# MatejBevec/gcn-song-embeddings

Hardware: AMD Instinct MI355X
Metric: PinSAGE train-step nodes/sec (2-hop, batch 512) at 1/2/4/8 MI355X (higher is better)
Workload: dtype f32

## Files before the change

gcn-song-embeddings_amd/csrc/capi.hip:

```cpp
#include <hip/hip_runtime.h>

#include <algorithm>
#include <cstdlib>
#include <cstring>
#include <string>
#include <vector>

#include "../../include/pinsage_hip.h"
#include "aggw.h"
#include "als.h"
#include "bpr.h"
#include "lmf.h"
#include "n2v.h"
#include "sage.h"
#include "capi.h"
#include "conv.h"
#include "cooc.h"
#include "dq.h"
#include "fly.h"
#include "frontier.h"
#include "gemm.h"
#include "knn.h"
#include "listmetrics.h"
#include "ppr_topk.h"
// ... 606 lines not shown
                 splits >= 0 && scratch && A3 && B3 && a3_ps >= 0 && b3_ps >= 0,
             kErrArg, "wgrad_planes: bad argument");
  KwParams p;
  p.A3 = A3;
  p.a3_ps = a3_ps;
  p.lda = lda;
  p.M = (int)M;
  p.B3 = B3;
  p.b3_ps = b3_ps;
  p.ldb = ldb;
  p.b_idx = b_idx;
  p.N = (int)N;
  p.K_dev = K_dev;
  p.K_max = (int)K_max;
  p.dst = dst;
  p.ld_dst = ld_dst;
  p.dst_b = dst_b;
  char* sc = static_cast<char*>(scratch);
  p.cnt = reinterpret_cast<int*>(sc);
  sc += align_up(wgrad_kw_tickets((int)M, (int)N) * 4, 256);
  p.slab = reinterpret_cast<float*>(sc);
  sc += wgrad_kw_slab_floats((int)M, (int)N) * 4;
  p.bslab = reinterpret_cast<float*>(sc);
  p.S = splits;
  return launch_wgrad_kw(p, (hipStream_t)stream);
}

int pinsage_gemm_ex(int64_t M, int64_t N, int64_t K, int a_kmajor, int b_kmajor, const float* A,
                    int64_t lda, const int32_t* a_idx, const float* B, int64_t ldb,
                    const int32_t* b_idx, float* C, int64_t ldc, const float* bias, int act,
                    int epi, int splits, int cfg, int stream_k, void* stream) {
  if (M < 0 || N <= 0 || K < 0 || M > INT32_MAX || N > INT32_MAX || K > INT32_MAX ||
      (epi != kEpiStore && epi != kEpiAccum && epi != kEpiPartial) || splits < 1 || cfg < -1 ||
      cfg > 5) {
    set_error("gemm_ex: bad argument");
    return kErrArg;
  }
  GemmParams p;
  p.M = (int)M;
  p.N = (int)N;
  p.K = (int)K;
  p.a_kmajor = a_kmajor != 0;
  p.b_kmajor = b_kmajor != 0;
  p.a = A;
  p.lda = lda;
  p.a_idx = a_idx;
  p.b = B;
  p.ldb = ldb;
  p.b_idx = b_idx;
  p.c = C;
  p.ldc = ldc;
  p.bias = bias;
  p.act = act != 0;
  p.epi = epi;
  p.splits = splits;
  p.cfg = cfg;
  p.stream_k = stream_k;
  if (cfg == 5 && (!gemm_ws_supported(p) || stream_k == 1 || gemm_default_prec() != 1)) {
    set_error("gemm_ex: cfg 5 needs split-bf16 products, K-major A and B, a store epilogue, K % 32 == 0, "
              "N % 128 == 0 and no stream-K");
    return kErrArg;
  }
  if (stream_k != 0) {
    static float* slab = nullptr;
    static int* cnt = nullptr;
    constexpr int64_t kCnt = 1 << 20;
    if (!slab) {
// ... 53 lines not shown
                       int64_t M_max, int64_t K, const float* W, const uint16_t* W_ilv, int64_t ldw_ilv,
                       const float* bias, int64_t N, int act, float* C, int64_t ldc, void* stream) {
  if (M < 0 || N <= 0 || K <= 0 || M > INT32_MAX || N > INT32_MAX || K > INT32_MAX || M_max < 0 ||
      M_max > INT32_MAX || (M_dev && M_max == 0)) {
    set_error("linear_ilv: bad argument");
    return kErrArg;
  }
  GemmParams p;
  p.M = (int)M;
  p.M_dev = M_dev;
  p.M_max = (int)M_max;
  p.N = (int)N;
  p.K = (int)K;
  p.a_ilv = A_ilv;
  p.lda_ilv = lda_ilv;
  p.a_idx = a_idx;
  p.b = W;
  p.ldb = K;
  p.b_ilv = W_ilv;
  p.ldb_ilv = W_ilv ? ldw_ilv : 0;
  p.c = C;
  p.ldc = ldc;
  p.bias = bias;
  p.act = act != 0;
  p.prec = 1;
  return launch_gemm(p, (hipStream_t)stream);
}

int pinsage_linear_split_b(const float* A, int64_t lda, const int32_t* a_idx, int64_t M, int64_t K,
                           const float* W, const uint16_t* W_planes, int64_t ldws,
                           const float* bias, int64_t N, int act, float* C, int64_t ldc, int cfg,
                           void* stream) {
  if (M < 0 || N <= 0 || K < 0 || M > INT32_MAX || N > INT32_MAX || K > INT32_MAX || cfg < -1 ||
      cfg > 5) {
    set_error("linear_split_b: bad argument");
    return kErrArg;
  }
  if (ldws != K) {
    set_error("linear_split_b: W_planes must come from pinsage_split_planes(W, N, K, ...): ldws == K");
    return kErrArg;
  }
  GemmParams p;
  p.M = (int)M;
  p.N = (int)N;
  p.K = (int)K;
  p.a = A;
  p.lda = lda;
  p.a_idx = a_idx;
  p.b = W;
  p.ldb = K;
  p.b_split = W_planes;
  p.ldb_split = ldws;
  p.c = C;
  p.ldc = ldc;
  p.bias = bias;
  p.act = act != 0;
  p.cfg = cfg;
  p.stream_k = 0;
  p.prec = 1;
  return launch_gemm(p, (hipStream_t)stream);
}

int64_t pinsage_cooc_tile(void) { return cooc_tile(); }

int64_t pinsage_cooc_scratch_bytes(int64_t n_tracks, int64_t batch_rows) {
  return cooc_scratch_bytes(n_tracks, batch_rows < 1 ? 1 : batch_rows);
}
// ... 307 lines not shown
  p.b = W;
  p.ldb = d + hid;
  p.c = y;
  p.ldc = out;
  p.bias = bias;
  p.epi = kEpiL2Norm;
  p.norms = norms;
  p.stream_k = 0;
  return launch_gemm(p, (hipStream_t)stream);
}

int pinsage_norm_lrelu_backward(const float* y, const float* norms, const float* dy, int64_t n, int64_t out,
                                float* dp, void* stream) {
  if (n < 0 || out <= 0 || out > INT32_MAX) {
    set_error("norm_lrelu_backward: bad sizes");
    return kErrArg;
  }
  if (n == 0) return kOk;
  return launch_norm_lrelu_bwd(y, norms, dy, (int)out, nullptr, n, dp, nullptr, 0, nullptr, nullptr, 0,
                               (hipStream_t)stream);
}

int64_t pinsage_gemm_sk_slab_floats(void) { return gemm_sk_slab_floats(); }

int pinsage_gemm_params(const pinsage_gemm_params_t* q, int* ran_stream_k, void* stream) {
  if (ran_stream_k) *ran_stream_k = 0;
  PS_REQUIRE(q && q->size == (int64_t)sizeof(pinsage_gemm_params_t), kErrArg,
             "gemm_params: null or a struct of another size");
  auto fits = [](int64_t v) { return v >= -1 && v <= INT32_MAX; };
  PS_REQUIRE(fits(q->M) && fits(q->N) && fits(q->K) && fits(q->M_max) && fits(q->K_max) && fits(q->K1) &&
                 fits(q->N1) && fits(q->splits) && fits(q->M_hint) && fits(q->sk_min_units) && q->M >= 0 &&
                 q->K >= 0 && q->M_max >= 0 && q->K_max >= 0 && q->splits >= 1 && q->M_hint >= 0,
             kErrArg, "gemm_params: a size out of range");
  PS_REQUIRE(q->epi >= kEpiStore && q->epi <= kEpiPartial && q->cfg >= -1 && q->cfg <= 5 && q->stream_k >= -1 &&
                 q->stream_k <= 1 && q->prec >= -1 && q->prec <= 1,
             kErrArg, "gemm_params: epi 0..3, cfg -1..5, stream_k -1..1, prec -1..1");
  PS_REQUIRE((q->a || q->a_ilv) && (q->b || q->b_ilv) && q->c, kErrArg, "gemm_params: a, b and c must be set");
  PS_REQUIRE((q->sk_slab != nullptr) == (q->sk_cnt != nullptr) && (!q->sk_cnt || q->sk_cnt_len > 0), kErrArg,
             "gemm_params: stream-K scratch needs the slab, the tickets and their count");
  GemmParams p;
  p.M = (int)q->M;
  p.N = (int)q->N;
  p.K = (int)q->K;
  p.M_dev = q->M_dev;
  p.K_dev = q->K_dev;
  p.M_max = (int)q->M_max;
  p.K_max = (int)q->K_max;
  p.a_kmajor = q->a_kmajor != 0;
  p.b_kmajor = q->b_kmajor != 0;
  p.a = q->a;
  p.lda = q->lda;
  p.a_idx = q->a_idx;
  p.K1 = (int)q->K1;
  p.a2 = q->a2;
  p.lda2 = q->lda2;
  p.a2_idx = q->a2_idx;
  p.b = q->b;
  p.ldb = q->ldb;
  p.b_idx = q->b_idx;
  p.N1 = (int)q->N1;
  p.b2 = q->b2;
  p.ldb2 = q->ldb2;
  p.b2_idx = q->b2_idx;
  p.c = q->c;
  p.ldc = q->ldc;
  p.c_idx = q->c_idx;
  p.c2 = q->c2;
  p.ldc2 = q->ldc2;
  p.bias_part = q->bias_part;
// ... 140 lines not shown
```

gcn-song-embeddings_amd/csrc/engine.hip:

```cpp
#include <hip/hip_runtime.h>

#include <algorithm>
#include <cstdlib>
#include <cstring>
#include <deque>
#include <functional>
#include <map>
#include <mutex>
#include <atomic>
#include <string>
#include <vector>

#include "aggw.h"
#include "common.h"
#include "conv.h"
#include "dq.h"
#include "frontier.h"
#include "gemm.h"
#include "head.h"
#include "wgrad.h"

namespace ps {

struct EngineConfig {
// ... 1173 lines not shown
  return kOk;
}

int pinsage_engine_read_counts(const pinsage_engine* e, void* ws, int64_t* S, int64_t* N,
                               void* stream) {
  const Engine* E = reinterpret_cast<const Engine*>(e);
  PS_CHECK_HIP(hipStreamSynchronize((hipStream_t)stream));
  for (size_t l = 0; l < E->L.size(); ++l) {
    int v = 0;
    PS_CHECK_HIP(hipMemcpy(&v, at<int>(ws, E->L[l].S.count), 4, hipMemcpyDeviceToHost));
    S[l] = v;
    PS_CHECK_HIP(hipMemcpy(&v, at<int>(ws, E->L[l].N.count), 4, hipMemcpyDeviceToHost));
    N[l] = v;
  }
  return kOk;
}

int pinsage_engine_set_frontier_fork(pinsage_engine* e, int on) {
  if (!e) {
    set_error("engine_set_frontier_fork: null engine");
    return kErrArg;
  }
  reinterpret_cast<Engine*>(e)->frontier_fork_ok = on != 0;
  return kOk;
}

int pinsage_engine_set_gemm_choice(pinsage_engine* e, const char* site, int cfg, int stream_k,
                                   int splits) {
  Engine* E = reinterpret_cast<Engine*>(e);
  if (!E || !site) {
    set_error("engine_set_gemm_choice: null argument");
    return kErrArg;
  }
  if (cfg < -1 || cfg > 5 || stream_k < -1 || stream_k > 1 || splits < 0 || splits > kMaxSplits) {
    set_error("engine_set_gemm_choice: cfg in [-1, 5], stream_k in [-1, 1], splits in [0, 64]");
    return kErrArg;
  }
  if (cfg < 0 && stream_k < 0 && splits == 0) E->choice.erase(site);
  else E->choice[site] = Engine::GemmChoice{cfg, stream_k, splits};
  return kOk;
}

int pinsage_engine_site_stream_k(const pinsage_engine* e, const char* site) {
  const Engine* E = reinterpret_cast<const Engine*>(e);
  if (!E || !site) return -1;
  auto it = E->sk_used.find(site);
  return it == E->sk_used.end() ? -1 : it->second;
}

int pinsage_engine_set_layer_table(pinsage_engine* e, int64_t layer, const int32_t* nb,
                                   const float* wn, int64_t ld) {
  Engine* E = reinterpret_cast<Engine*>(e);
  if (!E || layer < 0 || layer >= E->cfg.n_layers || ((nb == nullptr) != (wn == nullptr)) ||
      (nb && ld < E->cfg.T)) {
    set_error("engine_set_layer_table: bad argument");
    return kErrArg;
  }
  LayerBuf& lb = E->L[(size_t)layer];
  lb.nb_tab = nb;
  lb.wn_tab = wn;
  lb.ld_tab = ld;
  return kOk;
}

int pinsage_engine_set_hints(pinsage_engine* e, const int64_t* S, const int64_t* N) {
  Engine* E = reinterpret_cast<Engine*>(e);
  for (size_t l = 0; l < E->L.size(); ++l) {
    E->L[l].S.hint = S ? S[l] : 0;
// ... 191 lines not shown
```

gcn-song-embeddings_amd/csrc/gemm.h:

```cpp
#pragma once
#include "common.h"

namespace ps {

enum GemmEpi : int {
  kEpiStore = 0,
  kEpiAccum = 1,
  kEpiL2Norm = 2,
  kEpiPartial = 3,
};

struct GemmParams {
  int M = 0, N = 0, K = 0;
  const int* M_dev = nullptr;
  const int* K_dev = nullptr;
  int M_max = 0, K_max = 0;
  bool a_kmajor = true, b_kmajor = true;
  const float* a = nullptr;
  int64_t lda = 0;
  const int32_t* a_idx = nullptr;
  int K1 = -1;
  const float* a2 = nullptr;
  int64_t lda2 = 0;
  const int32_t* a2_idx = nullptr;
// ... 18 lines not shown
  float* norms = nullptr;
  int splits = 1;
  int M_hint = 0;
  int cfg = -1;
  float* sk_slab = nullptr;
  int* sk_cnt = nullptr;
  int64_t sk_cnt_len = 0;
  int stream_k = -1;
  int sk_min_units = 4;
  int prec = -1;
  const uint16_t* b_split = nullptr;
  int64_t ldb_split = 0;
  const uint16_t* a_ilv = nullptr;
  const uint16_t* b_ilv = nullptr;
  int64_t lda_ilv = 0, ldb_ilv = 0;
};

int launch_split_ilv(const float* src, int64_t ld, int64_t rows, int K, uint16_t* out, int64_t ldo, hipStream_t st);

int launch_split_planes(const float* w, int64_t rows, int64_t cols, int64_t ldw, uint16_t* out,
                        hipStream_t st);

int gemm_default_prec();
void gemm_set_default_prec(int prec);

int64_t gemm_sk_slab_floats();
int gemm_slots();

int gemm_pick_config(int M, int N, int K, int splits);

int launch_gemm(const GemmParams& p, hipStream_t st);
int gemm_last_stream_k();
bool gemm_ws_supported(const GemmParams& p);

}
```

gcn-song-embeddings_amd/csrc/gemm.hip:

```cpp
#include "gemm.h"

#include <algorithm>

#include "bf16split.h"
#include "lds_dma.h"
#include <type_traits>

namespace ps {

typedef float f32x16 __attribute__((ext_vector_type(16)));

constexpr int kLdsBudget = 81920;
constexpr int kLdsBudget3 = 54272;
constexpr int kLdsBudget4 = 40960;
constexpr int kIdxWin = 1024;

__device__ __forceinline__ void zero16(float* l) {
  *reinterpret_cast<float4*>(l) = make_float4(0.f, 0.f, 0.f, 0.f);
}

template <int R, int BK>
struct KOp {
  static constexpr int CPR = BK / 4;
  static constexpr int NI = R * CPR / 256;
  static constexpr int SZ = R * BK;
  static_assert(R * CPR % 256 == 0, "whole DMAs per thread");
  static constexpr int SH = BK == 32 ? 1 : 2;
  __device__ static __forceinline__ int swz(int row) { return (row >> SH) & (CPR - 1); }
  __device__ static __forceinline__ float4 frag(const float* img, int row, int k4) {
    return *reinterpret_cast<const float4*>(img + row * BK + 4 * ((k4 >> 2) ^ swz(row)));
  }
  const float* rp[NI];
  const float* rp2[NI];
  int lc[NI];
  __device__ __forceinline__ void init(int tid, int r0, int rmax, const float* a, int64_t lda,
                                       const int32_t* idx, const float* a2, int64_t lda2,
                                       const int32_t* idx2) {
#pragma unroll
    for (int j = 0; j < NI; ++j) {
      const int q = j * 256 + tid, row = q / CPR;
      lc[j] = 4 * ((q % CPR) ^ swz(row));
      const int g = r0 + row, rc = g < rmax ? g : rmax - 1;
      rp[j] = a + (int64_t)(idx ? idx[rc] : rc) * lda;
// ... 100 lines not shown
      base = a2 + (cl - c1);
      ld = lda2;
      gathered = idx2 != nullptr;
    } else {
      base = a + cl;
      ld = lda;
      gathered = idx != nullptr;
    }
  }
  __device__ __forceinline__ void issue(unsigned img, int wave, int k0, int kend, const int* sidx,
                                        int wb) const {
#pragma unroll
    for (int j = 0; j < NI; ++j) {
      const int k = min(k0 + kr0 + KSTEP * j, kend - 1);
      const int64_t r = gathered ? sidx[k - wb] : k;
      glds16(base + r * ld, img + (unsigned)(j * 256 + wave * 64) * 16u);
    }
  }
  __device__ __forceinline__ void zero_tail(float* img, int tid, int k0, int kend) const {
#pragma unroll
    for (int j = 0; j < NI; ++j)
      if (k0 + kr0 + KSTEP * j >= kend) zero16(img + (j * 256 + tid) * 4);
  }
};

struct SkPlan {
  int64_t U;
  int I, Ga;
  __device__ __forceinline__ int64_t start(int b) const { return (int64_t)b * U / Ga; }
  __device__ __forceinline__ int block_of(int64_t u) const {
    return (int)(((u + 1) * Ga - 1) / U);
  }
};

__device__ __forceinline__ float dpp_xor1(float x) {
  return __int_as_float(__builtin_amdgcn_mov_dpp(__float_as_int(x), 0xB1, 0xF, 0xF, false));
}
__device__ __forceinline__ float dpp_xor2(float x) {
  return __int_as_float(__builtin_amdgcn_mov_dpp(__float_as_int(x), 0x4E, 0xF, 0xF, false));
}
__device__ __forceinline__ void quad_transpose16(float (&v)[16], int lane) {
  const int i = lane & 3;
#pragma unroll
  for (int g = 0; g < 4; ++g) {
    float t[4];
#pragma unroll
    for (int k = 0; k < 4; ++k) t[k] = dpp_xor1(v[4 * g + (k ^ 1)]);
#pragma unroll
    for (int k = 0; k < 4; ++k)
      if ((i & 1) != (k & 1)) v[4 * g + k] = t[k];
#pragma unroll
    for (int k = 0; k < 4; ++k) t[k] = dpp_xor2(v[4 * g + (k ^ 2)]);
#pragma unroll
    for (int k = 0; k < 4; ++k)
      if ((i & 2) != (k & 2)) v[4 * g + k] = t[k];
  }
}

template <bool AK, bool BKM, int WM, int WN, int TM, int TN, int BK, int NSMAX = 4, int WPC = 2,
          bool BF = false, bool PB = false, bool SK = true, int IL = 0>
__global__ __launch_bounds__(256, WPC) void gemm_f32_kernel(GemmParams p) {
  static_assert(!BF || BK % 16 == 0, "split-bf16 products: 16-k steps");
  static_assert(!PB || (BF && BKM), "pre-split B: split-bf16 products, K-major B");
  static_assert(!IL || (BF && AK && BKM && !PB && !SK && BK == 16), "interleaved planes: split bf16, K-major A and B");
  constexpr int BM = WM * TM * 32, BN = WN * TN * 32;
  using OpA = typename std::conditional<
      IL != 0, IlvOp<BM>, typename std::conditional<AK, KOp<BM, BK>, MNOp<BM, BK>>::type>::type;
  using OpBp = typename std::conditional<
      PB, KSplitOp<BN, BK>, typename std::conditional<BKM, KOp<BN, BK>, MNOp<BN, BK>>::type>::type;
  using OpB = typename std::conditional<IL == 1, IlvOp<BN>, OpBp>::type;
  constexpr int SZA = OpA::SZ, SZB = OpB::SZ, SZS = SZA + SZB;
  constexpr int NG = OpA::NI + OpB::NI;
  constexpr bool GA = !AK, GB = !BKM;
  constexpr int IDXF = (GA ? kIdxWin : 0) + (GB ? kIdxWin : 0);
  constexpr int NSA = ((WPC == 2 ? kLdsBudget : WPC == 3 ? kLdsBudget3 : kLdsBudget4) / 4 - IDXF) / SZS;
  constexpr int NS = NSA > NSMAX ? NSMAX : NSA;
  static_assert(NS >= 3, "stage buffers do not fit");
  __shared__ __attribute__((aligned(16))) float smem[NS * SZS + IDXF];
  int* const sidxA = reinterpret_cast<int*>(smem + NS * SZS);
  int* const sidxB = sidxA + (GA ? kIdxWin : 0);

  const int tid = threadIdx.x, lane = tid & 63, wave = tid >> 6;
  const int wm = wave / WN, wn = wave % WN;
#ifdef PS_GEMM_PROBE
  uint64_t pt[6] = {__builtin_amdgcn_s_memrealtime(), 0, 0, 0, 0, 0};
  int pti = 1;
#define PS_PROBE() do { if (pti < 6) pt[pti++] = __builtin_amdgcn_s_memrealtime(); } while (0)
#else
#define PS_PROBE() do { } while (0)
#endif
// ... 275 lines not shown
          for (int o = 1; o < 32; o <<= 1) s2 += __shfl_xor(s2, o, 64);
          if (l32 == 0) red[wn * BM + (wm * TM + i) * 32 + (r & 3) + 8 * (r >> 2) + 4 * h] = s2;
        }
      __syncthreads();
#pragma unroll
      for (int i = 0; i < TM; ++i) {
        int64_t dsts[16];
#pragma unroll
        for (int r = 0; r < 16; ++r) {
          const int row = m0 + (wm * TM + i) * 32 + (r & 3) + 8 * (r >> 2) + 4 * h;
          dsts[r] = row < M ? (p.c_idx ? (int64_t)p.c_idx[row] : (int64_t)row) : -1;
        }
#pragma unroll
        for (int r = 0; r < 16; ++r) asm volatile("" : "+v"(dsts[r]));
#pragma unroll
        for (int r = 0; r < 16; ++r) {
          const int lrow = (wm * TM + i) * 32 + (r & 3) + 8 * (r >> 2) + 4 * h;
          const int row = m0 + lrow;
          if (row >= M) continue;
          float tot = 0.f;
#pragma unroll
          for (int q = 0; q < WN; ++q) tot += red[q * BM + lrow];
          const float nrm = sqrtf(tot);
          const int64_t dst = dsts[r];
#pragma unroll
          for (int j = 0; j < TN; ++j) {
            const int col = n0 + (wn * TN + j) * 32 + l32;
            if (col < N) p.c[dst * p.ldc + col] = acc[i][j][r] / nrm;
          }
          if (p.norms && wn == 0 && l32 == 0) p.norms[row] = nrm;
        }
      }
    } else {
      const bool accum = p.epi == kEpiAccum;
      const bool wide = N % 4 == 0 && p.ldc % 4 == 0 && (reinterpret_cast<uintptr_t>(p.c) & 15) == 0 &&
                        (!p.c2 || (p.ldc2 % 4 == 0 && p.N1 % 4 == 0 && (reinterpret_cast<uintptr_t>(p.c2) & 15) == 0)) &&
                        (!p.mask || (p.ldm % 4 == 0 && (reinterpret_cast<uintptr_t>(p.mask) & 15) == 0));
      if (wide) {
#pragma unroll
        for (int i = 0; i < TM; ++i)
#pragma unroll
          for (int j = 0; j < TN; ++j) {
            float v[16];
#pragma unroll
            for (int r = 0; r < 16; ++r) {
              float x = acc[i][j][r] + bj[j];
              if (p.act) x = lrelu(x);
              v[r] = x;
            }
            quad_transpose16(v, lane);
            const int col = n0 + (wn * TN + j) * 32 + 4 * (l32 >> 2);
            const bool second = p.c2 && col >= p.N1;
            int rows[4];
            int64_t dst[4];
#pragma unroll
            for (int g = 0; g < 4; ++g) {
              rows[g] = m0 + (wm * TM + i) * 32 + (l32 & 3) + 8 * g + 4 * h;
              dst[g] = rows[g] < M && col < N ? (p.c_idx ? (int64_t)p.c_idx[rows[g]] : (int64_t)rows[g]) : -1;
            }
            float4 pre[4];
#pragma unroll
            for (int g = 0; g < 4; ++g) {
              pre[g] = make_float4(0.f, 0.f, 0.f, 0.f);
              if (dst[g] >= 0) {
                if (p.mask) pre[g] = *reinterpret_cast<const float4*>(p.mask + (int64_t)rows[g] * p.ldm + col);
                else if (accum && !second) pre[g] = *reinterpret_cast<const float4*>(p.c + dst[g] * p.ldc + col);
              }
            }
            float4 val[4];
#pragma unroll
            for (int g = 0; g < 4; ++g) {
              float4 x = make_float4(v[4 * g], v[4 * g + 1], v[4 * g + 2], v[4 * g + 3]);
              if (p.mask) {
                x.x *= lrelu_grad(pre[g].x);
                x.y *= lrelu_grad(pre[g].y);
                x.z *= lrelu_grad(pre[g].z);
                x.w *= lrelu_grad(pre[g].w);
              } else if (accum && !second) {
                x.x = pre[g].x + x.x;
                x.y = pre[g].y + x.y;
                x.z = pre[g].z + x.z;
                x.w = pre[g].w + x.w;
              }
              val[g] = x;
              asm volatile("" : "+v"(val[g].x), "+v"(val[g].y), "+v"(val[g].z), "+v"(val[g].w));
            }
#pragma unroll
            for (int g = 0; g < 4; ++g)
              if (dst[g] >= 0)
                *reinterpret_cast<float4*>(second ? p.c2 + (int64_t)rows[g] * p.ldc2 + (col - p.N1)
                                                  : p.c + dst[g] * p.ldc + col) = val[g];
          }
      } else {
#pragma unroll
      for (int i = 0; i < TM; ++i)
#pragma unroll
        for (int r0 = 0; r0 < 16; r0 += 8) {
          int dsts[8];
#pragma unroll
          for (int r = 0; r < 8; ++r) {
            const int row = m0 + (wm * TM + i) * 32 + ((r0 + r) & 3) + 8 * ((r0 + r) >> 2) + 4 * h;
            dsts[r] = row < M ? (p.c_idx ? p.c_idx[row] : row) : -1;
          }
          float pre[8][TN];
#pragma unroll
          for (int r = 0; r < 8; ++r) {
            const int row = m0 + (wm * TM + i) * 32 + ((r0 + r) & 3) + 8 * ((r0 + r) >> 2) + 4 * h;
#pragma unroll
            for (int j = 0; j < TN; ++j) {
              const int col = n0 + (wn * TN + j) * 32 + l32;
              const bool ok = dsts[r] >= 0 && col < N;
              float x = 0.f;
              if (p.mask) x = ok ? lrelu_grad(p.mask[(int64_t)row * p.ldm + col]) : 0.f;
              else if (accum && !(p.c2 && col >= p.N1)) x = ok ? p.c[(int64_t)dsts[r] * p.ldc + col] : 0.f;
              pre[r][j] = x;
            }
          }
          float val[8][TN];
          float* rowp[8];
#pragma unroll
          for (int r = 0; r < 8; ++r) {
            rowp[r] = p.c + (int64_t)(dsts[r] < 0 ? 0 : dsts[r]) * p.ldc;
            asm volatile("" : "+v"(rowp[r]));
#pragma unroll
            for (int j = 0; j < TN; ++j) {
              const int col = n0 + (wn * TN + j) * 32 + l32;
              float v = acc[i][j][r0 + r] + bj[j];
              if (p.act) v = lrelu(v);
              if (p.mask) v *= pre[r][j];
              else if (accum && !(p.c2 && col >= p.N1)) v = pre[r][j] + v;
              val[r][j] = v;
              asm volatile("" : "+v"(val[r][j]));
            }
          }
#pragma unroll
          for (int r = 0; r < 8; ++r) {
            const int row = m0 + (wm * TM + i) * 32 + ((r0 + r) & 3) + 8 * ((r0 + r) >> 2) + 4 * h;
            if (row >= M) continue;
#pragma unroll
            for (int j = 0; j < TN; ++j) {
              const int col = n0 + (wn * TN + j) * 32 + l32;
              if (col >= N) continue;
              float* o = p.c2 && col >= p.N1 ? p.c2 + (int64_t)row * p.ldc2 + (col - p.N1) : rowp[r] + col;
              *o = val[r][j];
            }
          }
        }
      }
    }
    asm volatile("s_waitcnt lgkmcnt(0)" ::: "memory");
    __builtin_amdgcn_s_barrier();
    PS_PROBE();
#ifdef PS_GEMM_PROBE
    if (blockIdx.x == 0 && tid == 0)
      printf("gemm probe [10ns]: init %d wait0 %d kloop %d epi %d\n", (int)(pt[1] - pt[0]), (int)(pt[2] - pt[1]),
             (int)(pt[3] - pt[2]), (int)(pt[4] - pt[3]));
#endif
  };

  if constexpr (SK) if (p.sk_cnt) {
    SkPlan sk;
    sk.I = (K + BK - 1) / BK;
    sk.U = (int64_t)tiles_m * tiles_n * sk.I;
    if (sk.U == 0) return;
    const int64_t ga = sk.U / p.sk_min_units;
    sk.Ga = (int)(ga < 1 ? 1 : (ga < (int64_t)gridDim.x ? ga : (int64_t)gridDim.x));
    if (sk.Ga >= 8) sk.Ga &= ~7;
    const int per = sk.Ga >= 8 ? sk.Ga / 8 : sk.Ga;
    const int b = sk.Ga >= 8 ? (int)(blockIdx.x % 8) * per + (int)(blockIdx.x / 8) : (int)blockIdx.x;
    if ((int)blockIdx.x >= sk.Ga) return;
    const int64_t u0 = sk.start(b), u1 = sk.start(b + 1);
    const int t_first = (int)(u0 / sk.I);
    for (int64_t u = u0; u < u1;) {
      const int t = (int)(u / sk.I), i0 = (int)(u - (int64_t)t * sk.I);
      const int i1 = (int)min((int64_t)sk.I, i0 + (u1 - u));
      const bool part = !(i0 == 0 && i1 == sk.I);
      run_item(t / tiles_n, t % tiles_n, 0, i0 * BK, min(K, i1 * BK), part ? t : -1,
               2 * b + (t == t_first ? 0 : 1), sk);
      u += i1 - i0;
    }
    return;
// ... 180 lines not shown
          }
        }
      }
      __syncthreads();
    }
  }
}

bool gemm_ws_supported(const GemmParams& p) {
  return p.a_kmajor && p.b_kmajor && p.K1 < 0 && !p.a2 && !p.c_idx && !p.c2 && !p.mask && !p.b_split &&
         p.epi == kEpiStore && !p.K_dev && p.K > 0 && p.K % 32 == 0 && p.N % kWsBN == 0 && p.lda % 4 == 0 &&
         p.ldb % 4 == 0;
}

static int launch_gemm_ws(const GemmParams& p, int Mmax, hipStream_t st) {
  constexpr int BK = 32, AHEAD = 3, WPC = 1;
  static bool prepared = false;
  const int lds = kWsSlots * WsGeom<BK>::Slot;
  if (!prepared) {
    PS_CHECK_HIP(hipFuncSetAttribute((const void*)gemm_ws_kernel<BK, AHEAD, WPC>,
                                     hipFuncAttributeMaxDynamicSharedMemorySize, lds));
    prepared = true;
  }
  const int tm = (Mmax + kWsBM - 1) / kWsBM;
  const int tiles = tm * (p.N / kWsBN);
  const int iters = 8 * ((tm + 7) / 8) * (p.N / kWsBN);
  int grid = std::min(std::max(tiles, 1), WPC * gemm_slots() / 2);
  grid = std::min(grid, iters);
  hipLaunchKernelGGL((gemm_ws_kernel<BK, AHEAD, WPC>), dim3(grid), dim3(512), lds, st, p);
  PS_CHECK_LAUNCH();
  return kOk;
}

constexpr int kCfgBM[6] = {128, 64, 32, 64, 64, 64};

static int g_prec = -1;
int gemm_default_prec() {
  if (g_prec < 0) g_prec = getenv("PINSAGE_GEMM_PREC") ? atoi(getenv("PINSAGE_GEMM_PREC")) : 1;
  return g_prec;
}
void gemm_set_default_prec(int prec) { g_prec = prec; }

int gemm_slots() {
  static const int slots = [] {
    int dev = 0, cus = 0;
    if (hipGetDevice(&dev) != hipSuccess ||
        hipDeviceGetAttribute(&cus, hipDeviceAttributeMultiprocessorCount, dev) != hipSuccess ||
        cus <= 0)
      cus = 256;
    return 2 * cus;
  }();
  return slots;
}

int64_t gemm_sk_slab_floats() { return (int64_t)gemm_slots() * 2 * 64 * 128; }

int gemm_pick_config(int M, int N, int K, int splits) {
  if (splits > 1) return 0;
  const int64_t tn = (N + 127) / 128;
  const int64_t cus = gemm_slots() / 2;
  const int64_t t64 = ((M + 63) / 64) * tn;
  if (t64 > 2 * cus && (t64 <= 3 * cus || K <= 256)) return 3;
  int best = 0;
  int64_t best_cost = -1;
  for (int c = 0; c < 3; ++c) {
    const int64_t tiles = ((M + kCfgBM[c] - 1) / kCfgBM[c]) * tn;
    const int64_t cost = ((tiles + 255) / 256) * kCfgBM[c];
// ... 144 lines not shown
  PS_REQUIRE(p.epi != kEpiPartial || (!p.M_dev && !p.c_idx), kErrArg,
             "gemm: split-K partials need a static M");
  PS_REQUIRE(p.sk_min_units >= 1, kErrArg, "gemm: sk_min_units must be positive");
  PS_REQUIRE(p.cfg != 4 || (p.a_kmajor && p.b_kmajor), kErrArg,
             "gemm: cfg 4 (four workgroups per CU) needs K-major A and B");
  if (p.a_ilv || p.b_ilv) {
    PS_REQUIRE(p.a_ilv && p.a_kmajor && p.b_kmajor && !p.K_dev && p.K % 16 == 0 && p.K1 < 0 &&
                   (p.epi == kEpiStore || p.epi == kEpiAccum) && !p.c2 && p.lda_ilv % 8 == 0 &&
                   p.lda_ilv >= 3LL * p.K && (uintptr_t)p.a_ilv % 16 == 0 &&
                   (p.b_ilv ? p.ldb_ilv % 8 == 0 && p.ldb_ilv >= 3LL * p.K && (uintptr_t)p.b_ilv % 16 == 0
                            : p.b != nullptr),
               kErrArg, "gemm: interleaved planes need A's table, static K % 16 == 0 and a store epilogue");
    g_last_sk = 0;
    const int tiles_m = (Mmax + 127) / 128, tiles_n = (p.N + 127) / 128;
    const int64_t iters = 8LL * ((tiles_m + 7) / 8) * tiles_n;
    const int grid = (int)((std::min<int64_t>(iters, 1024) + 7) / 8 * 8);
    if (p.b_ilv)
      hipLaunchKernelGGL((gemm_f32_kernel<true, true, 2, 2, 2, 2, 16, 4, 2, true, false, false, 1>), dim3(grid),
                         dim3(256), 0, st, p);
    else
      hipLaunchKernelGGL((gemm_f32_kernel<true, true, 2, 2, 2, 2, 16, 4, 2, true, false, false, 2>), dim3(grid),
                         dim3(256), 0, st, p);
    PS_CHECK_LAUNCH();
    return kOk;
  }
  if (p.cfg == 5) {
    if (gemm_ws_supported(p) && (p.prec == 1 || (p.prec < 0 && gemm_default_prec() == 1))) {
      g_last_sk = 0;
      return launch_gemm_ws(p, Mmax, st);
    }
    p.cfg = 3;
    p.stream_k = 0;
  }
  PS_REQUIRE(!p.b_split || (p.b_kmajor && p.ldb_split % 8 == 0 && p.ldb_split >= Kmax &&
                            (p.K_dev || p.K % 8 == 0) && (uintptr_t)p.b_split % 16 == 0),
             kErrArg, "gemm: pre-split B needs K-major B, K and ldb_split multiples of 8, 16-B aligned planes");
  if (p.prec < 0) p.prec = gemm_default_prec();
  const int splits = p.epi == kEpiPartial ? p.splits : 1;
  const int Mest = p.M_dev ? (p.M_hint > 0 ? std::min(p.M_hint, Mmax) : Mmax) : p.M;
  int cfg = p.cfg >= 0 ? p.cfg : gemm_pick_config(Mest, p.N, Kmax, splits);
  const int tiles_n = (p.N + 127) / 128;
  const int slots = gemm_slots();

  const bool sk_allowed =
      p.sk_slab && p.sk_cnt && p.stream_k != 0 && p.epi != kEpiPartial && !p.K_dev && p.K > 0 &&
      (p.a_kmajor || !p.a_idx) && (p.b_kmajor || (!p.b_idx && !p.b2_idx));
  bool sk = false;
  if (sk_allowed) {
    const int skc = p.stream_k == 1 ? (p.cfg >= 0 ? p.cfg : 1) : 2;
    const int64_t tiles_max = (int64_t)((Mmax + kCfgBM[skc] - 1) / kCfgBM[skc]) * tiles_n;
    if ((skc == 1 || skc == 2) && tiles_max <= p.sk_cnt_len) {
      if (p.stream_k == 1) {
        sk = true;
      } else if (p.cfg < 0) {
        const int64_t tiles = (int64_t)((Mest + kCfgBM[skc] - 1) / kCfgBM[skc]) * tiles_n;
        sk = p.K >= 512 && tiles <= slots / 2;
      }
      if (sk) cfg = skc;
    }
  }
  if (!sk) {
    p.sk_cnt = nullptr;
    p.sk_slab = nullptr;
  }
  g_last_sk = sk ? 1 : 0;
  const int BMc = kCfgBM[cfg];
// ... 21 lines not shown
```

Measured before the change: 4.195 million.

## Add weight-resident persistent GEMM config for small-K linear layers

Adds a new GEMM kernel (cfg 6) that keeps the whole B tile (128 columns by up to 128 K) resident in LDS. Each block loops persistently over M tiles, double-buffering the A tiles through LDS DMA, and computes with a bf16x3 split MFMA product. The existing store epilogue moves into a shared header so both kernels use it. It targets small-K GEMMs where reloading weights per tile and per-tile launch overhead dominate, but it only runs when a caller selects cfg 6.

New measurement: 4.057 million. 3.3% lower.

```diff
diff --git a/gcn-song-embeddings_amd/csrc/capi.hip b/gcn-song-embeddings_amd/csrc/capi.hip
--- a/gcn-song-embeddings_amd/csrc/capi.hip
+++ b/gcn-song-embeddings_amd/csrc/capi.hip
@@ -662,7 +662,7 @@
                     int epi, int splits, int cfg, int stream_k, void* stream) {
   if (M < 0 || N <= 0 || K < 0 || M > INT32_MAX || N > INT32_MAX || K > INT32_MAX ||
       (epi != kEpiStore && epi != kEpiAccum && epi != kEpiPartial) || splits < 1 || cfg < -1 ||
-      cfg > 5) {
+      cfg > 6) {
     set_error("gemm_ex: bad argument");
     return kErrArg;
   }
@@ -782,7 +782,7 @@
                            const float* bias, int64_t N, int act, float* C, int64_t ldc, int cfg,
                            void* stream) {
   if (M < 0 || N <= 0 || K < 0 || M > INT32_MAX || N > INT32_MAX || K > INT32_MAX || cfg < -1 ||
-      cfg > 5) {
+      cfg > 6) {
     set_error("linear_split_b: bad argument");
     return kErrArg;
   }
@@ -1156,9 +1156,9 @@
                  fits(q->N1) && fits(q->splits) && fits(q->M_hint) && fits(q->sk_min_units) && q->M >= 0 &&
                  q->K >= 0 && q->M_max >= 0 && q->K_max >= 0 && q->splits >= 1 && q->M_hint >= 0,
              kErrArg, "gemm_params: a size out of range");
-  PS_REQUIRE(q->epi >= kEpiStore && q->epi <= kEpiPartial && q->cfg >= -1 && q->cfg <= 5 && q->stream_k >= -1 &&
+  PS_REQUIRE(q->epi >= kEpiStore && q->epi <= kEpiPartial && q->cfg >= -1 && q->cfg <= 6 && q->stream_k >= -1 &&
                  q->stream_k <= 1 && q->prec >= -1 && q->prec <= 1,
-             kErrArg, "gemm_params: epi 0..3, cfg -1..5, stream_k -1..1, prec -1..1");
+             kErrArg, "gemm_params: epi 0..3, cfg -1..6, stream_k -1..1, prec -1..1");
   PS_REQUIRE((q->a || q->a_ilv) && (q->b || q->b_ilv) && q->c, kErrArg, "gemm_params: a, b and c must be set");
   PS_REQUIRE((q->sk_slab != nullptr) == (q->sk_cnt != nullptr) && (!q->sk_cnt || q->sk_cnt_len > 0), kErrArg,
              "gemm_params: stream-K scratch needs the slab, the tickets and their count");
diff --git a/gcn-song-embeddings_amd/csrc/engine.hip b/gcn-song-embeddings_amd/csrc/engine.hip
--- a/gcn-song-embeddings_amd/csrc/engine.hip
+++ b/gcn-song-embeddings_amd/csrc/engine.hip
@@ -1229,8 +1229,8 @@
     set_error("engine_set_gemm_choice: null argument");
     return kErrArg;
   }
-  if (cfg < -1 || cfg > 5 || stream_k < -1 || stream_k > 1 || splits < 0 || splits > kMaxSplits) {
-    set_error("engine_set_gemm_choice: cfg in [-1, 5], stream_k in [-1, 1], splits in [0, 64]");
+  if (cfg < -1 || cfg > 6 || stream_k < -1 || stream_k > 1 || splits < 0 || splits > kMaxSplits) {
+    set_error("engine_set_gemm_choice: cfg in [-1, 6], stream_k in [-1, 1], splits in [0, 64]");
     return kErrArg;
   }
   if (cfg < 0 && stream_k < 0 && splits == 0) E->choice.erase(site);
diff --git a/gcn-song-embeddings_amd/csrc/gemm.h b/gcn-song-embeddings_amd/csrc/gemm.h
--- a/gcn-song-embeddings_amd/csrc/gemm.h
+++ b/gcn-song-embeddings_amd/csrc/gemm.h
@@ -74,5 +74,7 @@
 int launch_gemm(const GemmParams& p, hipStream_t st);
 int gemm_last_stream_k();
 bool gemm_ws_supported(const GemmParams& p);
+bool gemm_wk_supported(const GemmParams& p);
+int launch_gemm_wk(const GemmParams& p, int Mmax, hipStream_t st);
 
 }
diff --git a/gcn-song-embeddings_amd/csrc/gemm.hip b/gcn-song-embeddings_amd/csrc/gemm.hip
--- a/gcn-song-embeddings_amd/csrc/gemm.hip
+++ b/gcn-song-embeddings_amd/csrc/gemm.hip
@@ -3,12 +3,12 @@
 #include <algorithm>
 
 #include "bf16split.h"
+#include "gemm_epi.h"
 #include "lds_dma.h"
 #include <type_traits>
 
 namespace ps {
 
-typedef float f32x16 __attribute__((ext_vector_type(16)));
 
 constexpr int kLdsBudget = 81920;
 constexpr int kLdsBudget3 = 54272;
@@ -175,30 +175,6 @@
     return (int)(((u + 1) * Ga - 1) / U);
   }
 };
-
-__device__ __forceinline__ float dpp_xor1(float x) {
-  return __int_as_float(__builtin_amdgcn_mov_dpp(__float_as_int(x), 0xB1, 0xF, 0xF, false));
-}
-__device__ __forceinline__ float dpp_xor2(float x) {
-  return __int_as_float(__builtin_amdgcn_mov_dpp(__float_as_int(x), 0x4E, 0xF, 0xF, false));
-}
-__device__ __forceinline__ void quad_transpose16(float (&v)[16], int lane) {
-  const int i = lane & 3;
-#pragma unroll
-  for (int g = 0; g < 4; ++g) {
-    float t[4];
-#pragma unroll
-    for (int k = 0; k < 4; ++k) t[k] = dpp_xor1(v[4 * g + (k ^ 1)]);
-#pragma unroll
-    for (int k = 0; k < 4; ++k)
-      if ((i & 1) != (k & 1)) v[4 * g + k] = t[k];
-#pragma unroll
-    for (int k = 0; k < 4; ++k) t[k] = dpp_xor2(v[4 * g + (k ^ 2)]);
-#pragma unroll
-    for (int k = 0; k < 4; ++k)
-      if ((i & 2) != (k & 2)) v[4 * g + k] = t[k];
-  }
-}
 
 template <bool AK, bool BKM, int WM, int WN, int TM, int TN, int BK, int NSMAX = 4, int WPC = 2,
           bool BF = false, bool PB = false, bool SK = true, int IL = 0>
@@ -540,121 +516,7 @@
         }
       }
     } else {
-      const bool accum = p.epi == kEpiAccum;
-      const bool wide = N % 4 == 0 && p.ldc % 4 == 0 && (reinterpret_cast<uintptr_t>(p.c) & 15) == 0 &&
-                        (!p.c2 || (p.ldc2 % 4 == 0 && p.N1 % 4 == 0 && (reinterpret_cast<uintptr_t>(p.c2) & 15) == 0)) &&
-                        (!p.mask || (p.ldm % 4 == 0 && (reinterpret_cast<uintptr_t>(p.mask) & 15) == 0));
-      if (wide) {
-#pragma unroll
-        for (int i = 0; i < TM; ++i)
-#pragma unroll
-          for (int j = 0; j < TN; ++j) {
-            float v[16];
-#pragma unroll
-            for (int r = 0; r < 16; ++r) {
-              float x = acc[i][j][r] + bj[j];
-              if (p.act) x = lrelu(x);
-              v[r] = x;
-            }
-            quad_transpose16(v, lane);
-            const int col = n0 + (wn * TN + j) * 32 + 4 * (l32 >> 2);
-            const bool second = p.c2 && col >= p.N1;
-            int rows[4];
-            int64_t dst[4];
-#pragma unroll
-            for (int g = 0; g < 4; ++g) {
-              rows[g] = m0 + (wm * TM + i) * 32 + (l32 & 3) + 8 * g + 4 * h;
-              dst[g] = rows[g] < M && col < N ? (p.c_idx ? (int64_t)p.c_idx[rows[g]] : (int64_t)rows[g]) : -1;
-            }
-            float4 pre[4];
-#pragma unroll
-            for (int g = 0; g < 4; ++g) {
-              pre[g] = make_float4(0.f, 0.f, 0.f, 0.f);
-              if (dst[g] >= 0) {
-                if (p.mask) pre[g] = *reinterpret_cast<const float4*>(p.mask + (int64_t)rows[g] * p.ldm + col);
-                else if (accum && !second) pre[g] = *reinterpret_cast<const float4*>(p.c + dst[g] * p.ldc + col);
-              }
-            }
-            float4 val[4];
-#pragma unroll
-            for (int g = 0; g < 4; ++g) {
-              float4 x = make_float4(v[4 * g], v[4 * g + 1], v[4 * g + 2], v[4 * g + 3]);
-              if (p.mask) {
-                x.x *= lrelu_grad(pre[g].x);
-                x.y *= lrelu_grad(pre[g].y);
-                x.z *= lrelu_grad(pre[g].z);
-                x.w *= lrelu_grad(pre[g].w);
-              } else if (accum && !second) {
-                x.x = pre[g].x + x.x;
-                x.y = pre[g].y + x.y;
-                x.z = pre[g].z + x.z;
-                x.w = pre[g].w + x.w;
-              }
-              val[g] = x;
-              asm volatile("" : "+v"(val[g].x), "+v"(val[g].y), "+v"(val[g].z), "+v"(val[g].w));
-            }
-#pragma unroll
-            for (int g = 0; g < 4; ++g)
-              if (dst[g] >= 0)
-                *reinterpret_cast<float4*>(second ? p.c2 + (int64_t)rows[g] * p.ldc2 + (col - p.N1)
-                                                  : p.c + dst[g] * p.ldc + col) = val[g];
-          }
-      } else {
-#pragma unroll
-      for (int i = 0; i < TM; ++i)
-#pragma unroll
-        for (int r0 = 0; r0 < 16; r0 += 8) {
-          int dsts[8];
-#pragma unroll
-          for (int r = 0; r < 8; ++r) {
-            const int row = m0 + (wm * TM + i) * 32 + ((r0 + r) & 3) + 8 * ((r0 + r) >> 2) + 4 * h;
-            dsts[r] = row < M ? (p.c_idx ? p.c_idx[row] : row) : -1;
-          }
-          float pre[8][TN];
-#pragma unroll
-          for (int r = 0; r < 8; ++r) {
-            const int row = m0 + (wm * TM + i) * 32 + ((r0 + r) & 3) + 8 * ((r0 + r) >> 2) + 4 * h;
-#pragma unroll
-            for (int j = 0; j < TN; ++j) {
-              const int col = n0 + (wn * TN + j) * 32 + l32;
-              const bool ok = dsts[r] >= 0 && col < N;
-              float x = 0.f;
-              if (p.mask) x = ok ? lrelu_grad(p.mask[(int64_t)row * p.ldm + col]) : 0.f;
-              else if (accum && !(p.c2 && col >= p.N1)) x = ok ? p.c[(int64_t)dsts[r] * p.ldc + col] : 0.f;
-              pre[r][j] = x;
-            }
-          }
-          float val[8][TN];
-          float* rowp[8];
-#pragma unroll
-          for (int r = 0; r < 8; ++r) {
-            rowp[r] = p.c + (int64_t)(dsts[r] < 0 ? 0 : dsts[r]) * p.ldc;
-            asm volatile("" : "+v"(rowp[r]));
-#pragma unroll
-            for (int j = 0; j < TN; ++j) {
-              const int col = n0 + (wn * TN + j) * 32 + l32;
-              float v = acc[i][j][r0 + r] + bj[j];
-              if (p.act) v = lrelu(v);
-              if (p.mask) v *= pre[r][j];
-              else if (accum && !(p.c2 && col >= p.N1)) v = pre[r][j] + v;
-              val[r][j] = v;
-              asm volatile("" : "+v"(val[r][j]));
-            }
-          }
-#pragma unroll
-          for (int r = 0; r < 8; ++r) {
-            const int row = m0 + (wm * TM + i) * 32 + ((r0 + r) & 3) + 8 * ((r0 + r) >> 2) + 4 * h;
-            if (row >= M) continue;
-#pragma unroll
-            for (int j = 0; j < TN; ++j) {
-              const int col = n0 + (wn * TN + j) * 32 + l32;
-              if (col >= N) continue;
-              float* o = p.c2 && col >= p.N1 ? p.c2 + (int64_t)row * p.ldc2 + (col - p.N1) : rowp[r] + col;
-              *o = val[r][j];
-            }
-          }
-        }
-      }
+      gemm_epilogue_store<TM, TN>(p, acc, bj, m0, n0, M, N, wm, wn, lane);
     }
     asm volatile("s_waitcnt lgkmcnt(0)" ::: "memory");
     __builtin_amdgcn_s_barrier();
@@ -901,7 +763,7 @@
   return kOk;
 }
 
-constexpr int kCfgBM[6] = {128, 64, 32, 64, 64, 64};
+constexpr int kCfgBM[7] = {128, 64, 32, 64, 64, 64, 64};
 
 static int g_prec = -1;
 int gemm_default_prec() {
@@ -1112,6 +974,14 @@
     p.cfg = 3;
     p.stream_k = 0;
   }
+  if (p.cfg == 6) {
+    if (gemm_wk_supported(p) && (p.prec == 1 || (p.prec < 0 && gemm_default_prec() == 1))) {
+      g_last_sk = 0;
+      return launch_gemm_wk(p, Mmax, st);
+    }
+    p.cfg = 1;
+    p.stream_k = 0;
+  }
   PS_REQUIRE(!p.b_split || (p.b_kmajor && p.ldb_split % 8 == 0 && p.ldb_split >= Kmax &&
                             (p.K_dev || p.K % 8 == 0) && (uintptr_t)p.b_split % 16 == 0),
              kErrArg, "gemm: pre-split B needs K-major B, K and ldb_split multiples of 8, 16-B aligned planes");
diff --git a/gcn-song-embeddings_amd/csrc/gemm_epi.h b/gcn-song-embeddings_amd/csrc/gemm_epi.h
--- /dev/null
+++ b/gcn-song-embeddings_amd/csrc/gemm_epi.h
@@ -0,0 +1,154 @@
+#pragma once
+#include "gemm.h"
+
+namespace ps {
+
+typedef float f32x16 __attribute__((ext_vector_type(16)));
+
+__device__ __forceinline__ float dpp_xor1(float x) {
+  return __int_as_float(__builtin_amdgcn_mov_dpp(__float_as_int(x), 0xB1, 0xF, 0xF, false));
+}
+__device__ __forceinline__ float dpp_xor2(float x) {
+  return __int_as_float(__builtin_amdgcn_mov_dpp(__float_as_int(x), 0x4E, 0xF, 0xF, false));
+}
+__device__ __forceinline__ void quad_transpose16(float (&v)[16], int lane) {
+  const int i = lane & 3;
+#pragma unroll
+  for (int g = 0; g < 4; ++g) {
+    float t[4];
+#pragma unroll
+    for (int k = 0; k < 4; ++k) t[k] = dpp_xor1(v[4 * g + (k ^ 1)]);
+#pragma unroll
+    for (int k = 0; k < 4; ++k)
+      if ((i & 1) != (k & 1)) v[4 * g + k] = t[k];
+#pragma unroll
+    for (int k = 0; k < 4; ++k) t[k] = dpp_xor2(v[4 * g + (k ^ 2)]);
+#pragma unroll
+    for (int k = 0; k < 4; ++k)
+      if ((i & 2) != (k & 2)) v[4 * g + k] = t[k];
+  }
+}
+
+template <int TM, int TN>
+__device__ __forceinline__ void gemm_epilogue_store(const GemmParams& p, f32x16 (&acc)[TM][TN],
+                                                    const float (&bj)[TN], int m0, int n0, int M, int N,
+                                                    int wm, int wn, int lane) {
+  const int h = lane >> 5, l32 = lane & 31;
+  const bool accum = p.epi == kEpiAccum;
+  const bool wide = N % 4 == 0 && p.ldc % 4 == 0 && (reinterpret_cast<uintptr_t>(p.c) & 15) == 0 &&
+                    (!p.c2 || (p.ldc2 % 4 == 0 && p.N1 % 4 == 0 && (reinterpret_cast<uintptr_t>(p.c2) & 15) == 0)) &&
+                    (!p.mask || (p.ldm % 4 == 0 && (reinterpret_cast<uintptr_t>(p.mask) & 15) == 0));
+  if (wide) {
+#pragma unroll
+    for (int i = 0; i < TM; ++i)
+#pragma unroll
+      for (int j = 0; j < TN; ++j) {
+        float v[16];
+#pragma unroll
+        for (int r = 0; r < 16; ++r) {
+          float x = acc[i][j][r] + bj[j];
+          if (p.act) x = lrelu(x);
+          v[r] = x;
+        }
+        quad_transpose16(v, lane);
+        const int col = n0 + (wn * TN + j) * 32 + 4 * (l32 >> 2);
+        const bool second = p.c2 && col >= p.N1;
+        int rows[4];
+        int64_t dst[4];
+#pragma unroll
+        for (int g = 0; g < 4; ++g) {
+          rows[g] = m0 + (wm * TM + i) * 32 + (l32 & 3) + 8 * g + 4 * h;
+          dst[g] = rows[g] < M && col < N ? (p.c_idx ? (int64_t)p.c_idx[rows[g]] : (int64_t)rows[g]) : -1;
+        }
+        float4 pre[4];
+#pragma unroll
+        for (int g = 0; g < 4; ++g) {
+          pre[g] = make_float4(0.f, 0.f, 0.f, 0.f);
+          if (dst[g] >= 0) {
+            if (p.mask) pre[g] = *reinterpret_cast<const float4*>(p.mask + (int64_t)rows[g] * p.ldm + col);
+            else if (accum && !second) pre[g] = *reinterpret_cast<const float4*>(p.c + dst[g] * p.ldc + col);
+          }
+        }
+        float4 val[4];
+#pragma unroll
+        for (int g = 0; g < 4; ++g) {
+          float4 x = make_float4(v[4 * g], v[4 * g + 1], v[4 * g + 2], v[4 * g + 3]);
+          if (p.mask) {
+            x.x *= lrelu_grad(pre[g].x);
+            x.y *= lrelu_grad(pre[g].y);
+            x.z *= lrelu_grad(pre[g].z);
+            x.w *= lrelu_grad(pre[g].w);
+          } else if (accum && !second) {
+            x.x = pre[g].x + x.x;
+            x.y = pre[g].y + x.y;
+            x.z = pre[g].z + x.z;
+            x.w = pre[g].w + x.w;
+          }
+          val[g] = x;
+          asm volatile("" : "+v"(val[g].x), "+v"(val[g].y), "+v"(val[g].z), "+v"(val[g].w));
+        }
+#pragma unroll
+        for (int g = 0; g < 4; ++g)
+          if (dst[g] >= 0)
+            *reinterpret_cast<float4*>(second ? p.c2 + (int64_t)rows[g] * p.ldc2 + (col - p.N1)
+                                              : p.c + dst[g] * p.ldc + col) = val[g];
+      }
+  } else {
+#pragma unroll
+  for (int i = 0; i < TM; ++i)
+#pragma unroll
+    for (int r0 = 0; r0 < 16; r0 += 8) {
+      int dsts[8];
+#pragma unroll
+      for (int r = 0; r < 8; ++r) {
+        const int row = m0 + (wm * TM + i) * 32 + ((r0 + r) & 3) + 8 * ((r0 + r) >> 2) + 4 * h;
+        dsts[r] = row < M ? (p.c_idx ? p.c_idx[row] : row) : -1;
+      }
+      float pre[8][TN];
+#pragma unroll
+      for (int r = 0; r < 8; ++r) {
+        const int row = m0 + (wm * TM + i) * 32 + ((r0 + r) & 3) + 8 * ((r0 + r) >> 2) + 4 * h;
+#pragma unroll
+        for (int j = 0; j < TN; ++j) {
+          const int col = n0 + (wn * TN + j) * 32 + l32;
+          const bool ok = dsts[r] >= 0 && col < N;
+          float x = 0.f;
+          if (p.mask) x = ok ? lrelu_grad(p.mask[(int64_t)row * p.ldm + col]) : 0.f;
+          else if (accum && !(p.c2 && col >= p.N1)) x = ok ? p.c[(int64_t)dsts[r] * p.ldc + col] : 0.f;
+          pre[r][j] = x;
+        }
+      }
+      float val[8][TN];
+      float* rowp[8];
+#pragma unroll
+      for (int r = 0; r < 8; ++r) {
+        rowp[r] = p.c + (int64_t)(dsts[r] < 0 ? 0 : dsts[r]) * p.ldc;
+        asm volatile("" : "+v"(rowp[r]));
+#pragma unroll
+        for (int j = 0; j < TN; ++j) {
+          const int col = n0 + (wn * TN + j) * 32 + l32;
+          float v = acc[i][j][r0 + r] + bj[j];
+          if (p.act) v = lrelu(v);
+          if (p.mask) v *= pre[r][j];
+          else if (accum && !(p.c2 && col >= p.N1)) v = pre[r][j] + v;
+          val[r][j] = v;
+          asm volatile("" : "+v"(val[r][j]));
+        }
+      }
+#pragma unroll
+      for (int r = 0; r < 8; ++r) {
+        const int row = m0 + (wm * TM + i) * 32 + ((r0 + r) & 3) + 8 * ((r0 + r) >> 2) + 4 * h;
+        if (row >= M) continue;
+#pragma unroll
+        for (int j = 0; j < TN; ++j) {
+          const int col = n0 + (wn * TN + j) * 32 + l32;
+          if (col >= N) continue;
+          float* o = p.c2 && col >= p.N1 ? p.c2 + (int64_t)row * p.ldc2 + (col - p.N1) : rowp[r] + col;
+          *o = val[r][j];
+        }
+      }
+    }
+  }
+}
+
+}
diff --git a/gcn-song-embeddings_amd/csrc/gemm_wk.hip b/gcn-song-embeddings_amd/csrc/gemm_wk.hip
--- /dev/null
+++ b/gcn-song-embeddings_amd/csrc/gemm_wk.hip
@@ -0,0 +1,241 @@
+#include <algorithm>
+
+#include "bf16split.h"
+#include "gemm.h"
+#include "gemm_epi.h"
+#include "lds_dma.h"
+
+namespace ps {
+
+constexpr int kWkBM = 64, kWkBN = 128, kWkK = 128;
+constexpr int kWkNA = kWkBM * (kWkK / 4) / 256;
+constexpr int kWkNB = kWkBN * (kWkK / 4) / 256;
+constexpr int kWkSzA = kWkBM * kWkK, kWkSzB = kWkBN * kWkK;
+constexpr int kWkLds = (kWkSzB + 2 * kWkSzA) * 4;
+static_assert(kWkNB + 2 * kWkNA <= 63, "vmcnt counts every DMA in flight");
+
+__device__ __forceinline__ float4 wk_kfrag(const float* img, int row, int k4) {
+  return *reinterpret_cast<const float4*>(img + row * kWkK + 4 * ((k4 >> 2) ^ (row & 31)));
+}
+__device__ __forceinline__ int wk_kchunk_k(int tid, int j) {
+  return 4 * ((tid & 31) ^ ((j * 8 + (tid >> 5)) & 31));
+}
+
+template <bool BKM>
+__global__ __launch_bounds__(256, 1) void gemm_wk_kernel(GemmParams p, int P) {
+  extern __shared__ __attribute__((aligned(16))) float wk_lds[];
+  float* const sB = wk_lds;
+  float* const sA = wk_lds + kWkSzB;
+  const unsigned lds0 = (unsigned)(size_t)((__attribute__((address_space(3))) float*)wk_lds);
+  const int tid = threadIdx.x, lane = tid & 63, wave = tid >> 6;
+  const int wm = wave >> 1, wn = wave & 1;
+  const int h = lane >> 5, l32 = lane & 31;
+#ifdef PS_GEMM_PROBE
+  uint64_t pt[8] = {__builtin_amdgcn_s_memrealtime(), 0, 0, 0, 0, 0, 0, 0};
+  int pti = 1;
+#define PS_WK_PROBE() do { if (pti < 8) pt[pti++] = __builtin_amdgcn_s_memrealtime(); } while (0)
+#else
+#define PS_WK_PROBE() do { } while (0)
+#endif
+  const int M = p.M_dev ? *p.M_dev : p.M;
+  const int N = p.N, K = p.K;
+  const int tiles_m = (M + kWkBM - 1) / kWkBM, tiles_n = (N + kWkBN - 1) / kWkBN;
+  int pw, tn;
+  if ((P & 7) == 0) {
+    const int x = blockIdx.x & 7, s = blockIdx.x >> 3;
+    pw = (s / tiles_n) * 8 + x;
+    tn = s % tiles_n;
+  } else {
+    pw = blockIdx.x % P;
+    tn = blockIdx.x / P;
+  }
+  if (pw >= tiles_m || tn >= tiles_n) return;
+  const int n0 = tn * kWkBN;
+  const int nsteps = (K + 15) / 16, K16 = nsteps * 16;
+
+  auto a_rows = [&](int tm, const float* (&rp)[kWkNA]) __attribute__((always_inline)) {
+#pragma unroll
+    for (int j = 0; j < kWkNA; ++j) {
+      const int g = tm * kWkBM + j * 8 + (tid >> 5), rc = g < M ? g : M - 1;
+      rp[j] = p.a + (int64_t)(p.a_idx ? p.a_idx[rc] : rc) * p.lda;
+    }
+  };
+  auto a_issue = [&](int buf, const float* const (&rp)[kWkNA]) __attribute__((always_inline)) {
+    const unsigned img = lds0 + (unsigned)(kWkSzB + buf * kWkSzA) * 4u;
+#pragma unroll
+    for (int j = 0; j < kWkNA; ++j)
+      glds16(rp[j] + min(wk_kchunk_k(tid, j), K - 4), img + (unsigned)(j * 256 + wave * 64) * 16u);
+  };
+  auto a_zero_tail = [&](int buf) __attribute__((always_inline)) {
+    if (K == K16) return;
+#pragma unroll
+    for (int j = 0; j < kWkNA; ++j)
+      if (wk_kchunk_k(tid, j) >= K) *reinterpret_cast<float4*>(sA + buf * kWkSzA + (j * 256 + tid) * 4) =
+          make_float4(0.f, 0.f, 0.f, 0.f);
+  };
+
+  const float* rp[kWkNA];
+  const float* rn[kWkNA];
+  const bool more = pw + P < tiles_m;
+  a_rows(pw, rp);
+  if (more) a_rows(pw + P, rn);
+  float bj[2];
+#pragma unroll
+  for (int j = 0; j < 2; ++j) {
+    const int col = n0 + (wn * 2 + j) * 32 + l32;
+    bj[j] = (p.bias && col < N) ? p.bias[col] : 0.f;
+    asm volatile("" : "+v"(bj[j]));
+  }
+#pragma unroll
+  for (int j = 0; j < kWkNA; ++j) {
+    asm volatile("" : "+v"(rp[j]));
+    if (more) asm volatile("" : "+v"(rn[j]));
+  }
+  if constexpr (BKM) {
+#pragma unroll
+    for (int j = 0; j < kWkNB; ++j) {
+      const int g = n0 + j * 8 + (tid >> 5), rc = g < N ? g : N - 1;
+      glds16(p.b + (int64_t)rc * p.ldb + min(wk_kchunk_k(tid, j), K - 4),
+             lds0 + (unsigned)(j * 256 + wave * 64) * 16u);
+    }
+  } else {
+    const int cc = n0 + 4 * (tid & 31), cl = cc < N ? cc : N - 4;
+#pragma unroll
+    for (int j = 0; j < kWkNB; ++j) {
+      if (8 * j >= K16) continue;
+      const int k = min(j * 8 + (tid >> 5), K - 1);
+      glds16(p.b + (int64_t)k * p.ldb + cl, lds0 + (unsigned)(j * 256 + wave * 64) * 16u);
+    }
+  }
+  a_issue(0, rp);
+  if (more) {
+    a_issue(1, rn);
+    asm volatile("s_waitcnt vmcnt(%0)" ::"n"(kWkNA) : "memory");
+  } else {
+    asm volatile("s_waitcnt vmcnt(0)" ::: "memory");
+  }
+  if (K != K16) {
+    if constexpr (BKM) {
+#pragma unroll
+      for (int j = 0; j < kWkNB; ++j)
+        if (wk_kchunk_k(tid, j) >= K) *reinterpret_cast<float4*>(sB + (j * 256 + tid) * 4) =
+            make_float4(0.f, 0.f, 0.f, 0.f);
+    } else {
+#pragma unroll
+      for (int j = 0; j < kWkNB; ++j)
+        if (8 * j < K16 && j * 8 + (tid >> 5) >= K) *reinterpret_cast<float4*>(sB + (j * 256 + tid) * 4) =
+            make_float4(0.f, 0.f, 0.f, 0.f);
+    }
+    a_zero_tail(0);
+  }
+  PS_WK_PROBE();
+  asm volatile("s_waitcnt lgkmcnt(0)" ::: "memory");
+  __builtin_amdgcn_s_barrier();
+  PS_WK_PROBE();
+
+  int it = 0;
+  for (int tm = pw; tm < tiles_m; tm += P, ++it) {
+    const float* As = sA + (it & 1) * kWkSzA;
+    const bool has1 = tm + P < tiles_m, has2 = tm + 2 * P < tiles_m;
+    if (has2) a_rows(tm + 2 * P, rn);
+
+    f32x16 acc[1][2];
+#pragma unroll
+    for (int j = 0; j < 2; ++j)
+#pragma unroll
+      for (int r = 0; r < 16; ++r) acc[0][j][r] = 0.f;
+    const int ar = wm * 32 + l32;
+    struct Frag {
+      bf16x8 aH, aM, aL, bH[2], bM[2], bL[2];
+    };
+    auto fetch = [&](int t, Frag& f) __attribute__((always_inline)) {
+      const int k8 = 16 * t + 8 * h;
+      split3(wk_kfrag(As, ar, k8), wk_kfrag(As, ar, k8 + 4), f.aH, f.aM, f.aL);
+#pragma unroll
+      for (int j = 0; j < 2; ++j) {
+        const int c = (wn * 2 + j) * 32 + l32;
+        if constexpr (BKM) {
+          split3(wk_kfrag(sB, c, k8), wk_kfrag(sB, c, k8 + 4), f.bH[j], f.bM[j], f.bL[j]);
+        } else {
+          const float* b0 = sB + k8 * kWkBN + c;
+          split3(make_float4(b0[0], b0[kWkBN], b0[2 * kWkBN], b0[3 * kWkBN]),
+                 make_float4(b0[4 * kWkBN], b0[5 * kWkBN], b0[6 * kWkBN], b0[7 * kWkBN]), f.bH[j], f.bM[j],
+                 f.bL[j]);
+        }
+      }
+    };
+    auto products = [&](const Frag& f) __attribute__((always_inline)) {
+#define PS_WK2(X, Y)                                                                    \
+  acc[0][0] = __builtin_amdgcn_mfma_f32_32x32x16_bf16(f.X, f.Y[0], acc[0][0], 0, 0, 0); \
+  acc[0][1] = __builtin_amdgcn_mfma_f32_32x32x16_bf16(f.X, f.Y[1], acc[0][1], 0, 0, 0);
+      PS_WK2(aL, bH)
+      PS_WK2(aH, bL)
+      PS_WK2(aM, bM)
+      PS_WK2(aM, bH)
+      PS_WK2(aH, bM)
+      PS_WK2(aH, bH)
+#undef PS_WK2
+    };
+    if (nsteps == kWkK / 16) {
+      Frag f[2];
+      fetch(0, f[0]);
+#pragma unroll
+      for (int t = 0; t < kWkK / 16; ++t) {
+        if (t + 1 < kWkK / 16) fetch(t + 1, f[(t + 1) & 1]);
+        products(f[t & 1]);
+      }
+    } else {
+      for (int t = 0; t < nsteps; ++t) {
+        Frag f;
+        fetch(t, f);
+        products(f);
+      }
+    }
+    PS_WK_PROBE();
+    if (has1) {
+      asm volatile("s_waitcnt vmcnt(0)" ::: "memory");
+      a_zero_tail((it + 1) & 1);
+      asm volatile("s_waitcnt lgkmcnt(0)" ::: "memory");
+      __builtin_amdgcn_s_barrier();
+      if (has2) a_issue(it & 1, rn);
+    }
+    PS_WK_PROBE();
+    gemm_epilogue_store<1, 2>(p, acc, bj, tm * kWkBM, n0, M, N, wm, wn, lane);
+    PS_WK_PROBE();
+  }
+#ifdef PS_GEMM_PROBE
+  if (blockIdx.x == 0 && tid == 0)
+    printf("gemm_wk probe [10ns]: issue %d fill %d | kloop %d swap %d epi %d | kloop %d swap %d epi %d\n",
+           (int)(pt[1] - pt[0]), (int)(pt[2] - pt[1]), (int)(pt[3] - pt[2]), (int)(pt[4] - pt[3]),
+           (int)(pt[5] - pt[4]), (int)(pt[6] - pt[5]), (int)(pt[7] - pt[6]), 0);
+#endif
+}
+
+bool gemm_wk_supported(const GemmParams& p) {
+  return p.a_kmajor && p.a && p.b && !p.K_dev && p.K >= 4 && p.K <= kWkK && p.K % 4 == 0 && p.K1 < 0 && !p.a2 &&
+         !p.b2 && !p.b_idx && !p.b2_idx && !p.b_split && !p.a_ilv && !p.b_ilv &&
+         (p.epi == kEpiStore || p.epi == kEpiAccum) && (p.b_kmajor || p.N >= 4) && p.lda % 4 == 0 &&
+         p.ldb % 4 == 0 && (reinterpret_cast<uintptr_t>(p.a) & 15) == 0 && (reinterpret_cast<uintptr_t>(p.b) & 15) == 0;
+}
+
+int launch_gemm_wk(const GemmParams& p, int Mmax, hipStream_t st) {
+  static bool prepared = false;
+  if (!prepared) {
+    PS_CHECK_HIP(hipFuncSetAttribute((const void*)gemm_wk_kernel<true>, hipFuncAttributeMaxDynamicSharedMemorySize,
+                                     kWkLds));
+    PS_CHECK_HIP(hipFuncSetAttribute((const void*)gemm_wk_kernel<false>, hipFuncAttributeMaxDynamicSharedMemorySize,
+                                     kWkLds));
+    prepared = true;
+  }
+  const int cus = gemm_slots() / 2;
+  const int tiles_m = (Mmax + kWkBM - 1) / kWkBM, tiles_n = (p.N + kWkBN - 1) / kWkBN;
+  int P = std::max(1, std::min(tiles_m, cus / tiles_n));
+  if (P >= 8) P &= ~7;
+  const int grid = P * tiles_n;
+  if (p.b_kmajor) hipLaunchKernelGGL(gemm_wk_kernel<true>, dim3(grid), dim3(256), kWkLds, st, p, P);
+  else hipLaunchKernelGGL(gemm_wk_kernel<false>, dim3(grid), dim3(256), kWkLds, st, p, P);
+  PS_CHECK_LAUNCH();
+  return kOk;
+}
+
+}
```
